# timoblak/sq-recovery

Hardware: AMD Instinct MI355X
Metric: training images/sec (256x256 depth, implicit loss) (higher is better)
Workload: dtype bf16; 1 GPU; ResNetSQ + ImplicitLoss(R=32, tau=1.5, s=260) train step, Adam; model=ResNetSQ (resnet18 backbone, 11.37M params), global_batch=64, per_gpu_batch=64, image=256x256x1, render_size=32, parallelism=dp1

## Files before the change

sq-recovery_amd/csrc/sqr_conv3.hip:

```cpp
#include <stdint.h>
#include <stdlib.h>
#include <type_traits>
#include "sqr_conv_dev.h"

namespace sqr {
namespace conv {

#ifdef SQR_STAMPS
#ifndef SQR_STAMP_MAXWG
#define SQR_STAMP_MAXWG 8192
#endif
#define SQR_STAMP_DECL unsigned long long stamp_[5] = {0, 0, 0, 0, 0};
#define SQR_STAMP(i) (stamp_[i] = wall_clock64())
#define SQR_STAMP_WRITE(tp)                                                              \
  do {                                                                                   \
    if ((tp) && threadIdx.x == 0 && blockIdx.x < SQR_STAMP_MAXWG) {                      \
      for (int i_ = 0; i_ < 5; ++i_) (tp)[2 + 8 * blockIdx.x + i_] = stamp_[i_];          \
      (tp)[2 + 8 * blockIdx.x + 5] = blockIdx.x;                                         \
    }                                                                                    \
  } while (0)
#else
#define SQR_STAMP_DECL
#define SQR_STAMP(i) ((void)0)
#define SQR_STAMP_WRITE(tp) ((void)0)
#endif

__device__ __forceinline__ int d3key(int row) { return row & 6; }

constexpr unsigned long long K20_LUT = 0xadc1f8859b07e93ull;
__device__ __forceinline__ int k20key(int row) { return (int)((K20_LUT >> (3 * (row % 20))) & 7); }

struct D3Args {
  const void* x;
  const void* w;
  void* out;
  const void* addend;
  const uint8_t* addend_mask;
  const void* bn_x;
  const uint8_t* bn_mask;
  const float* bn_mean;
  const float* bn_coef;
  void* bn_act;
  const float* in_coef;
  float* stats;
  int N, H, W, Cin, Nout;
  int iH, iW;
  int tiles_x, tiles_per_img;
  int ntm, ntn;
  int flip;
  uint32_t xbytes, wbytes;
  unsigned long long* tp;
#ifdef SQR_EXPERIMENTS
  int exp;
#endif
};

#ifdef SQR_EXPERIMENTS
#define SQR_ABL(a, bit) (((a).exp & (bit)) != 0)
#else
#define SQR_ABL(a, bit) false
#endif

__device__ __forceinline__ void dma_piece(__amdgpu_buffer_rsrc_t srd, char* dst, uint32_t voff, int soff) {
  __builtin_amdgcn_raw_ptr_buffer_load_lds(srd, (__attribute__((address_space(3))) void*)dst, 16, voff, soff, 0, 0);
}

template <int PIECES, int NW>
__device__ __forceinline__ void dma_pieces(__amdgpu_buffer_rsrc_t srd, char* dst, const uint32_t* voff, int soff,
                                           int wave) {
#pragma unroll
  for (int i = 0; i < PIECES; ++i)
    __builtin_amdgcn_raw_ptr_buffer_load_lds(srd, (__attribute__((address_space(3))) void*)(dst + ((i * NW + wave) * 8) * 128),
                                             16, voff[i], soff, 0, 0);
}

template <int BN, int WAVES_M, int WAVES_N, int TN, int NT>
__device__ __forceinline__ void stats_reduce(const float (*s1)[4], const float (*s2)[4], float* red, int wm, int wn,
                                             int fr, int fq, int tid, float* stats_row0, float* stats_row1) {
  constexpr int WN = BN / WAVES_N;
  float* r1 = red + (wm * 16 + fr) * BN + wn * WN + 4 * fq;
  float* r2 = r1 + WAVES_M * 16 * BN;
#pragma unroll
  for (int j = 0; j < TN; ++j) {
    *(f32x4*)(r1 + 16 * j) = f32x4{s1[j][0], s1[j][1], s1[j][2], s1[j][3]};
    *(f32x4*)(r2 + 16 * j) = f32x4{s2[j][0], s2[j][1], s2[j][2], s2[j][3]};
  }
  __syncthreads();
  for (int c = tid; c < 2 * BN; c += NT) {
    const int q = c / BN, col = c - q * BN;
    const float* src = red + q * WAVES_M * 16 * BN + col;
    float acc = 0.f;
#pragma unroll 8
    for (int r = 0; r < WAVES_M * 16; ++r) acc += src[r * BN];
    (q ? stats_row1 : stats_row0)[col] = acc;
  }
}

template <typename T, int BN, int WAVES_M, int WAVES_N, int TM, int TN, int NT>
__device__ __forceinline__ void tile_stats(const uint32_t (*pk)[TM][2], float* red, int wm, int wn, int fr, int fq,
                                           int tid, float* stats_row0, float* stats_row1, float* count, float bm) {
  constexpr int WN = BN / WAVES_N;
  constexpr float NG = 16.f * TM, INV_NG = 1.f / (16.f * TM);
  float* r1 = red + wm * BN + wn * WN + 4 * fq;
  float* r2 = r1 + WAVES_M * BN;
  float m[TN][4], q[TN][4];
#pragma unroll
  for (int j = 0; j < TN; ++j) {
#pragma unroll
    for (int e = 0; e < 4; ++e) {
      float v[TM];
#pragma unroll
      for (int i = 0; i < TM; ++i) v[i] = (e & 1) ? hi2f<T>(pk[j][i][e >> 1]) : lo2f<T>(pk[j][i][e >> 1]);
      const float K = row_first(v[0]);
      float sa = 0.f, sq = 0.f;
#pragma unroll
      for (int i = 0; i < TM; ++i) {
        const float d = v[i] - K;
        sa += d;
        sq = fmaf(d, d, sq);
      }
      sa = row_sum15(sa);
      sq = row_sum15(sq);
      const float sn = sa * INV_NG;
      m[j][e] = K + sn;
      q[j][e] = fmaxf(sq - sa * sn, 0.f);
    }
  }
  if (fr == 15) {
#pragma unroll
    for (int j = 0; j < TN; ++j) {
      *(f32x4*)(r1 + 16 * j) = f32x4{m[j][0], m[j][1], m[j][2], m[j][3]};
      *(f32x4*)(r2 + 16 * j) = f32x4{q[j][0], q[j][1], q[j][2], q[j][3]};
    }
  }
  __syncthreads();
  for (int col = tid; col < BN; col += NT) {
    float mean, m2;
    lane_rows_merge(red + col, red + WAVES_M * BN + col, WAVES_M, BN, NG, &mean, &m2);
    stats_row0[col] = mean;
    stats_row1[col] = m2;
  }
  if (count && tid == 0) *count = bm;
}

#ifndef SQR_D3_WINPF
#define SQR_D3_WINPF 1
#endif
template <typename T, int BM, int BN, int WAVES_M, int WAVES_N, int TW, int TH, int NWB, int IMGS = 1, int PD = 2,
          bool ACC = false, bool BNB = false, int S = 1, bool BNIN = false>
__global__ void __launch_bounds__(64 * WAVES_M * WAVES_N) conv3_kernel(D3Args a) {
  constexpr int NT = 64 * WAVES_M * WAVES_N, NW = WAVES_M * WAVES_N;
  constexpr int ROWB = 128, STAGES = PD + 1;
  constexpr int WM = BM / WAVES_M, WN = BN / WAVES_N;
  constexpr int TM = WM / 16, TN = WN / 16;
  static_assert(S == 1 || (S == 2 && IMGS == 1 && !ACC && !BNB), "stride 2: forward, one image per tile");
  constexpr int WWID = S == 1 ? TW + 2 : TW + 1;
  static_assert(!BNIN || (S == 1 && !ACC && !BNB), "apply-on-load: stride-1 forward");
  constexpr bool K20 = S == 1 && TW == 8 && !BNIN;
  constexpr int P0 = (TH + 1) * WWID, P1 = TH * WWID;
  constexpr int WRI = S == 1 ? (TH + 2) * WWID : 2 * P0 + 2 * P1, WR = IMGS * WRI;
  constexpr int WROWS = (WR + 8 * NW - 1) / (8 * NW) * (8 * NW);
  constexpr int PB = BN / (8 * NW);
  constexpr int WP = WROWS / (8 * NW);
  static_assert(BM == IMGS * TH * TW, "pixel tile");
  static_assert(PB >= 1 && PB * 8 * NW == BN, "BN must be a multiple of 8 * waves");
  constexpr int WIN = WROWS * ROWB, TILE_B = BN * ROWB;
  constexpr int LDS = NWB * WIN + STAGES * TILE_B;
  static_assert(2 * WAVES_M * 16 * BN * 4 <= LDS, "stats scratch fits the ring");
  __shared__ __attribute__((aligned(1024))) char smem[LDS + (BNIN ? 2 * 512 * 4 : 0)];
  float* const ctab = (float*)(smem + LDS);
  char* const bring = smem + NWB * WIN;
  clock_begin(a.tp);
  SQR_STAMP_DECL
  SQR_STAMP(0);

  const int tid = threadIdx.x, lane = tid & 63;
  const int wave = __builtin_amdgcn_readfirstlane(tid >> 6);
  const int wm = wave / WAVES_N, wn = wave % WAVES_N;
  const int bid = xcd_remap(blockIdx.x, gridDim.x);
  const int tile_m = bid / a.ntn, tile_n = bid - (bid / a.ntn) * a.ntn;
  const int img = (tile_m / a.tiles_per_img) * IMGS;
  const int trem = tile_m - (tile_m / a.tiles_per_img) * a.tiles_per_img;
  const int ty = trem / a.tiles_x, tx = trem - ty * a.tiles_x;
  const int h0 = ty * TH, w0 = tx * TW, n0 = tile_n * BN;

  const int fr = lane & 15, fq = lane >> 4;
  auto out_off = [&](int i) -> size_t {
    const int m = wm * WM + 16 * i + fr;
    const int ii = m / (TH * TW), mm = m - ii * (TH * TW);
    return (((size_t)(img + ii) * a.H + h0 + mm / TW) * a.W + w0 + (mm % TW)) * a.Nout + n0 + wn * WN + 4 * fq;
  };
  u32x2 av[ACC || BNB ? TN : 1][ACC || BNB ? TM : 1];
  uint32_t bmk[(BNB || ACC) ? TN : 1][(BNB || ACC) ? TM : 1];
  constexpr bool LATE = NW == 4 && TM * TN >= 16;
  auto load_av = [&]() {
    const uint16_t* ad = (const uint16_t*)(BNB ? a.bn_x : a.addend);
#pragma unroll
    for (int i = 0; i < TM; ++i) {
      const size_t o = out_off(i);
#pragma unroll
      for (int j = 0; j < TN; ++j) {
        av[j][i] = *(const u32x2*)(ad + o + 16 * j);
        if constexpr (BNB) bmk[j][i] = a.bn_coef ? 0u : a.bn_mask[(o + 16 * j) >> 3];
        if constexpr (ACC) bmk[j][i] = a.addend_mask ? a.addend_mask[(o + 16 * j) >> 3] : 0xffu;
      }
    }
  };
  if constexpr ((ACC || BNB) && !LATE) load_av();

  constexpr uint32_t kOOB = 0x80000000u;
  const int prow = lane >> 3, pslot = lane & 7;
  uint32_t wvoff[WP];
#pragma unroll
  for (int i = 0; i < WP; ++i) {
    const int r = (i * NW + wave) * 8 + prow;
    const int ls = pslot ^ (K20 ? k20key(r) : d3key(r));
    const int ii = r / WRI, rr = r - ii * WRI;
    int h, w;
    bool used = r < WR;
    if constexpr (S == 1) {
      const int wy = rr / WWID, wx = rr - wy * WWID;
      h = h0 - 1 + wy;
      w = w0 - 1 + wx;
    } else {
      const int pa = rr >= 2 * P0 ? 1 : 0;
// ... 257 lines not shown
      pk[j][i][0] = pack2<T>(acc[j][i][0], acc[j][i][1]);
      pk[j][i][1] = pack2<T>(acc[j][i][2], acc[j][i][3]);
    }
  uint32_t ak[BNB ? TN : 1][BNB ? TM : 1][2];
  if constexpr (BNB) {
    const bool bc = a.bn_coef != nullptr;
    float s1[TN][4], s2[TN][4], mu[TN][4], csc[TN][4], csh[TN][4];
#pragma unroll
    for (int j = 0; j < TN; ++j)
#pragma unroll
      for (int e = 0; e < 4; ++e) {
        const int c = n0 + wn * WN + 16 * j + 4 * fq + e;
        s1[j][e] = s2[j][e] = 0.f;
        mu[j][e] = a.bn_mean[c];
        const float* cp = bc ? a.bn_coef : a.bn_mean;
        csc[j][e] = cp[c];
        csh[j][e] = cp[bc ? a.Nout + c : c];
      }
#pragma unroll
    for (int j = 0; j < TN; ++j)
#pragma unroll
      for (int i = 0; i < TM; ++i) {
        uint32_t mb;
        if (bc) {
          mb = 0;
#pragma unroll
          for (int h = 0; h < 2; ++h) {
            const uint32_t v = pack2<T>(fmaxf(fmaf(lo2f<T>(av[j][i][h]), csc[j][2 * h], csh[j][2 * h]), 0.f),
                                        fmaxf(fmaf(hi2f<T>(av[j][i][h]), csc[j][2 * h + 1], csh[j][2 * h + 1]), 0.f));
            ak[j][i][h] = v;
            mb |= (lo2f<T>(v) > 0.f ? 1u : 0u) << (2 * h);
            mb |= (hi2f<T>(v) > 0.f ? 1u : 0u) << (2 * h + 1);
          }
        } else {
          mb = (bmk[j][i] >> ((opix[i] + 16 * j) & 4)) & 0xfu;
        }
        pk[j][i][0] &= ((mb & 1u) ? 0xffffu : 0u) | ((mb & 2u) ? 0xffff0000u : 0u);
        pk[j][i][1] &= ((mb & 4u) ? 0xffffu : 0u) | ((mb & 8u) ? 0xffff0000u : 0u);
#pragma unroll
        for (int h = 0; h < 2; ++h) {
          const float g0 = lo2f<T>(pk[j][i][h]), g1 = hi2f<T>(pk[j][i][h]);
          s1[j][2 * h] += g0;
          s2[j][2 * h] = fmaf(g0, lo2f<T>(av[j][i][h]) - mu[j][2 * h], s2[j][2 * h]);
          s1[j][2 * h + 1] += g1;
          s2[j][2 * h + 1] = fmaf(g1, hi2f<T>(av[j][i][h]) - mu[j][2 * h + 1], s2[j][2 * h + 1]);
        }
      }
    stats_reduce<BN, WAVES_M, WAVES_N, TN, NT>(s1, s2, (float*)smem, wm, wn, fr, fq, tid,
                                               a.stats + ((size_t)tile_m * 2) * a.Nout + n0,
                                               a.stats + ((size_t)tile_m * 2 + 1) * a.Nout + n0);
  }
  uint16_t* out = (uint16_t*)a.out;
  static_assert(TN % 2 == 0, "tile pairs");
  const int sw = 12 * (fq & 1);
#pragma unroll
  for (int i = 0; i < TM; ++i)
#pragma unroll
    for (int j = 0; j < TN; j += 2) {
      const auto r0 = __builtin_amdgcn_permlane16_swap(pk[j][i][0], pk[j + 1][i][0], false, false);
      const auto r1 = __builtin_amdgcn_permlane16_swap(pk[j][i][1], pk[j + 1][i][1], false, false);
      if (!SQR_ABL(a, 2)) *(u32x4*)(out + opix[i] + 16 * j + sw) = u32x4{r0[0], r1[0], r0[1], r1[1]};
      if constexpr (BNB) {
        if (a.bn_act) {
          const auto q0 = __builtin_amdgcn_permlane16_swap(ak[j][i][0], ak[j + 1][i][0], false, false);
          const auto q1 = __builtin_amdgcn_permlane16_swap(ak[j][i][1], ak[j + 1][i][1], false, false);
          *(u32x4*)((uint16_t*)a.bn_act + opix[i] + 16 * j + sw) = u32x4{q0[0], q1[0], q0[1], q1[1]};
        }
      }
    }
  if (!BNB && a.stats)
    tile_stats<T, BN, WAVES_M, WAVES_N, TM, TN, NT>(pk, (float*)smem, wm, wn, fr, fq, tid,
                                                 a.stats + ((size_t)tile_m * 2) * a.Nout + n0,
                                                 a.stats + ((size_t)tile_m * 2 + 1) * a.Nout + n0,
                                                 tile_n == 0 ? a.stats + (size_t)a.ntm * 2 * a.Nout + tile_m : nullptr,
                                                 (float)BM);
#ifdef SQR_STAMPS
  asm volatile("s_waitcnt vmcnt(0)" ::: "memory");
#endif
  SQR_STAMP(4);
  SQR_STAMP_WRITE(a.tp);
  clock_end(a.tp);
}


struct D3PArgs {
  const void* x;
  const void* w;
  void* out;
  const void* addend;
  const uint8_t* addend_mask;
  const void* bn_x;
  const uint8_t* bn_mask;
  const float* bn_mean;
  float* stats;
  const float* in_coef;
  void* in_act;
  uint8_t* in_mask;
  int H, bpi, tpb, flip;
  uint32_t xbytes, wbytes;
  unsigned long long* tp;
};

template <typename T, bool STATS, bool ACC = false, bool BNB = false, int TW = 64, int TH = 2, bool BNIN = false>
__global__ void __launch_bounds__(256) conv3p_kernel(D3PArgs a) {
  constexpr int C = 64, BN = 64, NW = 4, NT = 256, ROWB = 128;
  constexpr int WAVES_M = 2, WAVES_N = 2, WM = TH * TW / WAVES_M, WN = 32, TM = WM / 32;
  constexpr int SLOTR = (TW + 2 + 7) / 8 * 8;
  constexpr int PPR = SLOTR / 8;
  constexpr int NSLOT = TH + 2 <= 4 ? 4 : 8;
  constexpr int RING = NSLOT * SLOTR * ROWB;
  constexpr int WB = 9 * BN * ROWB;
  constexpr int WPW = 9 * BN / (8 * NW);
  constexpr int STG = TH * TW * BN * 2;
  constexpr int NST = STG / 16 / NT;
  static_assert(TW % 32 == 0 && TM * 32 == WM && WN == 32, "a wave's pixels are whole 32-pixel runs of rows");
  static_assert(STG <= WB, "the staged tile fits the weight image's region");
  static_assert(2 * WAVES_M * 32 * BN * 4 <= RING && NT * 16 * 4 <= RING, "statistics scratch fits the ring");
  static_assert(NST <= 8, "store schedule");
  static_assert(!BNIN || (STATS && !ACC && !BNB), "apply-on-load: forward launches only");
  __shared__ __attribute__((aligned(1024))) char smem[WB + RING];
  __shared__ __attribute__((aligned(16))) float bnc[BNIN ? 128 : 4];
  char* const wl = smem + RING;
  char* const ring = smem;
  char* const stg = wl;
  clock_begin(a.tp);

  const int tid = threadIdx.x, lane = tid & 63;
  const int wave = __builtin_amdgcn_readfirstlane(tid >> 6);
  const int wm = wave / WAVES_N, wn = wave % WAVES_N;
  const int prow = lane >> 3, pslot = lane & 7;
  constexpr uint32_t kOOB = 0x80000000u;
  const __amdgpu_buffer_rsrc_t xsrd = __builtin_amdgcn_make_buffer_rsrc((void*)a.x, 0, a.xbytes, 0x00020000);
  const __amdgpu_buffer_rsrc_t wsrd = __builtin_amdgcn_make_buffer_rsrc((void*)a.w, 0, a.wbytes, 0x00020000);
  const int H = a.H, ntile = a.tpb;
  const int img = blockIdx.x / a.bpi;
  const int hb = (blockIdx.x - img * a.bpi) * ntile * TH;

  constexpr int RPW = (TH * PPR + NW - 1) / NW;
  constexpr int PRW = ((TH + 2) * PPR + NW - 1) / NW;
  auto row_piece = [&](int r0, int p, uint32_t* vo, bool use = true) {
    const int j = p / PPR, part = p - j * PPR;
    const int row = r0 + j;
    const int lbase = ((row + 1) & (NSLOT - 1)) * SLOTR + part * 8;
    const int L = lbase + prow, w = part * 8 + prow - 1;
    const bool ok = use && (unsigned)row < (unsigned)H && (unsigned)w < (unsigned)TW;
    *vo = ok ? (uint32_t)((((img * H + row) * TW + w) * C) * 2 + (pslot << 4)) : kOOB;
    return L * ROWB + ((pslot ^ ((L >> 1) & 7)) << 4);
  };
  auto load_rows = [&](int r0, int nrows, u32x4* v, bool use) {
#pragma unroll
    for (int i = 0; i < PRW; ++i) {
      const int p = i * NW + wave;
      if (i < (nrows * PPR + NW - 1) / NW) {
        uint32_t vo;
        row_piece(r0, p, &vo, use && p < nrows * PPR);
        v[i] = __builtin_amdgcn_raw_buffer_load_b128(xsrd, vo, 0, 0);
      }
    }
  };
  auto load_row_piece = [&](int r0, int i, u32x4* v, bool use) {
    const int p = i * NW + wave;
    uint32_t vo;
    row_piece(r0, p, &vo, use && p < TH * PPR);
    v[i] = __builtin_amdgcn_raw_buffer_load_b128(xsrd, vo, 0, 0);
  };
  auto write_rows = [&](int r0, int nrows, const u32x4* v) {
// ... 425 lines not shown
  const int H = 2 * a.Ho, W = 2 * a.Wo;
  T* out = (T*)a.dx;
  constexpr int NIT = (HALF + 64 * NW - 1) / (64 * NW), AG = NIT < 4 ? NIT : 4;
  static_assert(NIT % AG == 0, "addend groups");
  auto piece = [&](int it, int ph, int& p, int& sl, size_t& go) {
    const int idx = tid + it * 64 * NW;
    p = idx / SL;
    sl = idx - p * SL;
    const int y = p / PX, x = p - y * PX;
    go = (((size_t)img * H + 2 * (i0 + y) + ph) * W + 2 * j0 + x) * a.C + n0 + 8 * sl;
    return idx < HALF && i0 + y < a.Ho && j0 + (x >> 1) < a.Wo;
  };
  auto load_group = [&](int it0, int ph, uint4* av) {
#pragma unroll
    for (int u = 0; u < AG; ++u) {
      int p, sl;
      size_t go;
      if (piece(it0 + u, ph, p, sl, go)) {
        if (a.addend_s2) {
          const int y = p / PX, x = p - y * PX;
          av[u] = (x & 1) ? uint4{0u, 0u, 0u, 0u}
                          : *(const uint4*)((const T*)a.addend +
                                            (((size_t)img * a.Ho + i0 + y) * a.Wo + j0 + (x >> 1)) * a.C + n0 +
                                                8 * sl);
        } else {
          av[u] = *(const uint4*)((const T*)a.addend + go);
        }
      }
    }
  };
#pragma unroll
  for (int ph = 0; ph < 2; ++ph) {
    const bool add = a.addend && !(a.addend_s2 && ph == 1);
    uint4 av[AG];
    if (add) load_group(0, ph, av);
    if (ph) __syncthreads();
#pragma unroll
    for (int pw = 0; pw < 2; ++pw)
#pragma unroll
      for (int i = 0; i < TM; ++i) {
        const int m = wm * WM + 16 * i + fr;
        const int p = (m / TW) * PX + 2 * (m % TW) + pw;
#pragma unroll
        for (int j = 0; j < TN; ++j) {
          const int n = wn * WN + 16 * j + 4 * fq;
          const int slot = (n >> 3) ^ ((p >> 1) & 7);
          store4((T*)(smem + p * (BN * 2) + slot * 16 + (n & 4) * 2), acc[2 * ph + pw][j][i]);
        }
      }
    __syncthreads();
#pragma unroll
    for (int it0 = 0; it0 < NIT; it0 += AG) {
      if (it0 && add) load_group(it0, ph, av);
#pragma unroll
      for (int u = 0; u < AG; ++u) {
        int p, sl;
        size_t go;
        if (!piece(it0 + u, ph, p, sl, go)) continue;
        uint4 v = *(const uint4*)(smem + p * (BN * 2) + ((sl ^ ((p >> 1) & 7)) << 4));
        if (add) {
          uint32_t* vv = (uint32_t*)&v;
          const uint32_t* aa = (const uint32_t*)&av[u];
#pragma unroll
          for (int e = 0; e < 4; ++e)
            vv[e] = pack2<T>(lo2f<T>(vv[e]) + lo2f<T>(aa[e]), hi2f<T>(vv[e]) + hi2f<T>(aa[e]));
        }
        *(uint4*)(out + go) = v;
      }
    }
  }
  asm volatile("s_waitcnt vmcnt(0) lgkmcnt(0)" ::: "memory");
  clock_end(a.tp);
}

__device__ __forceinline__ int psw(int y, int x) { return ((x >> 1) & 1) | ((((x >> 3) ^ y) & 1) << 1); }

template <int OFF>
__device__ __forceinline__ s16x4 ds_read_tr16_off(uint32_t addr) {
  s16x4 r;
  asm volatile("ds_read_b64_tr_b16 %0, %1 offset:%2" : "=v"(r) : "v"(addr), "n"(OFF));
  return r;
}

template <int B, int E, typename F>
__device__ __forceinline__ void static_for(F&& f) {
  if constexpr (B < E) {
    f(std::integral_constant<int, B>{});
    static_for<B + 1, E>(f);
  }
}

template <int N>
__device__ __forceinline__ void lgkm_wait() {
  static_assert(N >= 0 && N <= 15, "lgkmcnt field");
  asm volatile("s_waitcnt lgkmcnt(%0)" ::"n"(N) : "memory");
}

template <int PER>
__device__ __forceinline__ void wait_vm_chunks(int m) {
  if (m >= 2) {
    asm volatile("s_waitcnt vmcnt(%0)" ::"n"(2 * PER) : "memory");
  } else if (m == 1) {
    asm volatile("s_waitcnt vmcnt(%0)" ::"n"(PER) : "memory");
  } else {
    asm volatile("s_waitcnt vmcnt(0)" ::: "memory");
  }
}

constexpr int wg_lgkm(int j, int D, int NS, bool last) {
  int n = 0;
  for (int k = j - D + 1; k <= j - 1; ++k) {
    if (last && k + D >= NS) continue;
    n += 2 + ((k + D) % 9 == 0 ? 8 : 0);
  }
  return n > 15 ? 15 : n;
}

struct D3WArgs {
  const void* x;
  const void* dy;
  float* slab;
  int N, H, W, C, K, Ho, Wo;
  int tiles_x, chunks_per_img, nchunks, cps;
  int ntc, ntiles;
  uint32_t xbytes, dybytes;
  unsigned long long* tp;
};

template <int S, int TW, int TH>
struct WgWin {
  static constexpr int PH(int a) { return S == 1 ? TH + 2 : TH + 1 - a; }
  static constexpr int PW(int b) { return S == 1 ? TW + 2 : (b ? TW : TW + 2); }
  static constexpr int PB(int a, int b) {
    return S == 1 ? 0 : (a * 2 + b >= 1 ? PH(0) * PW(0) : 0) + (a * 2 + b >= 2 ? PH(0) * PW(1) : 0) +
                            (a * 2 + b >= 3 ? PH(1) * PW(0) : 0);
  }
  static constexpr int ROWS = S == 1 ? PH(0) * PW(0) : PB(1, 1) + PH(1) * PW(1);
  static constexpr int YO(int r) { return S == 1 ? r : r >> 1; }
  static constexpr int PA(int r) { return S == 1 ? 0 : r & 1; }
};

template <typename T, int TW, int TH, int STAGES, int S>
__global__ void __launch_bounds__(256) conv3_wgrad_kernel(D3WArgs a) {
  constexpr int NW = 4, ROWB = 128;
  constexpr int BKP = TW * TH, SUBS = BKP / 32;
  using Win = WgWin<S, TW, TH>;
  constexpr int WR = Win::ROWS;
  constexpr int WROWS = (WR + 31) / 32 * 32;
  constexpr int DP = BKP / 32, XP = WROWS / 32;
  constexpr int PER = DP + XP;
  constexpr int TILE_D = BKP * ROWB, STAGE = TILE_D + WROWS * ROWB;
  static_assert(BKP % 64 == 0, "chunk = multiple of 64 pixels");
  __shared__ __attribute__((aligned(1024))) char smem[STAGES * STAGE];

  const int tid = threadIdx.x, lane = tid & 63;
  const int wave = __builtin_amdgcn_readfirstlane(tid >> 6);
  const int bid = xcd_remap(blockIdx.x, gridDim.x);
  clock_begin(a.tp);
  SQR_STAMP_DECL
  SQR_STAMP(0);
  const int split = bid / a.ntiles, tile = bid - split * a.ntiles;
  const int k0 = (tile / a.ntc) * 64, c0 = (tile % a.ntc) * 64;
  const int ch0 = split * a.cps;
  const int nloc = min(a.nchunks - ch0, a.cps);

  constexpr uint32_t kOOB = 0x80000000u;
  const int prow = lane >> 3, pslot = lane & 7;
  uint32_t dvoff[DP];
#pragma unroll
  for (int i = 0; i < DP; ++i) {
    const int r = (i * NW + wave) * 8 + prow;
    const int lch = 2 * ((pslot >> 1) ^ psw(r / TW, r % TW)) + (pslot & 1);
    dvoff[i] = (uint32_t)((((r / TW) * a.Wo + (r % TW)) * a.K + k0 + lch * 8) * 2);
  }
// ... 207 lines not shown
  clock_end(a.tp);
}

namespace {
int g_direct = 1;
int g_deep_ring = 1;

#ifdef SQR_EXPERIMENTS
int exp_env(const char* n, int dflt) {
  const char* v = getenv(n);
  return v && *v ? atoi(v) : dflt;
}
#else
constexpr int exp_env(const char*, int dflt) { return dflt; }
#endif

int pow2_log(int x) {
  int l = 0;
  while ((1 << l) < x) ++l;
  return (1 << l) == x ? l : -1;
}

int dt16(int dtype) { return dtype == SQR_DTYPE_F16 ? 1 : 0; }

using D3Launch = void (*)(dim3 grid, hipStream_t st, const D3Args& a);
struct D3Entries {
  D3Launch plain;
  D3Launch acc;
  D3Launch bnb;
  D3Launch bnin;
};
struct D3Tile {
  int id;
  int BN, WAVES_M, WAVES_N, TW, TH, NWB, IMGS, PD;
  bool exact_bn;
  bool deep_ring;
  bool nso_faster;
  D3Entries e[2];
};
enum : unsigned { kExactBn = 1, kDeepRing = 2, kNsoFaster = 4 };
constexpr int kNoBnin = -1, kBninSamePd = 0;

template <typename T, int BN, int WM, int WN, int TW, int TH, int NWB, int IMGS, int PD, bool ACC, bool BNB, int S,
          bool BNIN>
void d3_launch(dim3 grid, hipStream_t st, const D3Args& a) {
  hipLaunchKernelGGL((conv3_kernel<T, IMGS * TH * TW, BN, WM, WN, TW, TH, NWB, IMGS, PD, ACC, BNB, S, BNIN>), grid,
                     dim3(64 * WM * WN), 0, st, a);
}
template <typename T, int BN, int WM, int WN, int TW, int TH, int NWB, int IMGS, int PD, int BNIN_PD, int S>
constexpr D3Entries d3_entries() {
  D3Entries e = {d3_launch<T, BN, WM, WN, TW, TH, NWB, IMGS, PD, false, false, S, false>, nullptr, nullptr, nullptr};
  if constexpr (S == 1) {
    e.acc = d3_launch<T, BN, WM, WN, TW, TH, NWB, IMGS, PD, true, false, S, false>;
    e.bnb = d3_launch<T, BN, WM, WN, TW, TH, NWB, IMGS, PD, false, true, S, false>;
  }
  if constexpr (BNIN_PD != kNoBnin)
    e.bnin = d3_launch<T, BN, WM, WN, TW, TH, NWB, IMGS, BNIN_PD == kBninSamePd ? PD : BNIN_PD, false, false, S, true>;
  return e;
}
template <int ID, int BN, int WM, int WN, int TW, int TH, int NWB, int IMGS, int PD, int BNIN_PD = kNoBnin, int S = 1>
constexpr D3Tile d3_tile(unsigned flags = 0) {
  return {ID, BN, WM, WN, TW, TH, NWB, IMGS, PD, (flags & kExactBn) != 0, (flags & kDeepRing) != 0,
          (flags & kNsoFaster) != 0,
          {d3_entries<bf16, BN, WM, WN, TW, TH, NWB, IMGS, PD, BNIN_PD, S>(),
           d3_entries<f16, BN, WM, WN, TW, TH, NWB, IMGS, PD, BNIN_PD, S>()}};
}

constexpr D3Tile kD3Tiles[] = {
    d3_tile<0, 64, 4, 1, 64, 4, 1, 1, 2>(kExactBn),
    d3_tile<7, 128, 4, 2, 32, 8, 2, 1, 3, 2>(kDeepRing | kNsoFaster),
    d3_tile<8, 128, 4, 2, 16, 8, 2, 1, 5, kBninSamePd>(kDeepRing | kNsoFaster),
    d3_tile<10, 64, 2, 2, 8, 8, 2, 2, 8, kBninSamePd>(kDeepRing),
    d3_tile<1, 128, 4, 2, 32, 8, 2, 1, 2, kBninSamePd>(kNsoFaster),
    d3_tile<2, 128, 4, 2, 16, 8, 2, 1, 2, kBninSamePd>(kNsoFaster),
    d3_tile<5, 64, 2, 2, 8, 8, 2, 2, 2, kBninSamePd>(),
    d3_tile<3, 128, 2, 2, 8, 8, 2, 1, 2>(),
    d3_tile<4, 64, 4, 1, 16, 16, 2, 1, 2>(),
};
constexpr D3Tile kD3S2FTiles[] = {
    d3_tile<0, 128, 4, 2, 32, 4, 1, 1, 2, kNoBnin, 2>(),
    d3_tile<1, 128, 2, 2, 16, 4, 2, 1, 2, kNoBnin, 2>(),
    d3_tile<2, 128, 2, 2, 8, 8, 2, 1, 2, kNoBnin, 2>(),
};
constexpr int kBninMaxC = 512;

bool enough_tiles(long long tiles) { return !(tiles < 128 && g_direct < 2); }

const D3Tile* pick(int N, int H, int W, int Cin, int Nout) {
  const int nch = Cin / 64;
  static const int force = exp_env("SQR_D3_CFG", -1);
  for (const D3Tile& c : kD3Tiles) {
    if (force >= 0 && c.id != force) continue;
    if (force < 0 && !g_deep_ring && c.deep_ring) continue;
    if (c.exact_bn ? Nout != c.BN : Nout % c.BN) continue;
    if (W % c.TW || H % c.TH) continue;
    if (c.IMGS > 1 && (c.TH != H || c.TW != W || N % c.IMGS)) continue;
    if (c.NWB == 1 && nch != 1) continue;
    if (!enough_tiles((long long)(N / c.IMGS) * (H / c.TH) * (W / c.TW) * (Nout / c.BN))) continue;
    return &c;
  }
  return nullptr;
}

const D3Tile* pick_s2f(int N, int Ho, int Wo, int Cin, int Nout) {
  const int nch = Cin / 64;
  static const int force = exp_env("SQR_S2F_CFG", -1);
  for (const D3Tile& c : kD3S2FTiles) {
    if (force >= 0 && c.id != force) continue;
    if ((c.NWB == 1) != (nch == 1)) continue;
    if (Nout % c.BN || Wo % c.TW || Ho % c.TH) continue;
    if (!enough_tiles((long long)N * (Ho / c.TH) * (Wo / c.TW) * (Nout / c.BN))) continue;
    return &c;
  }
  return nullptr;
}

int persist_rows(int W) { return W == 64 ? 2 : 1; }
bool persist_shape(int Cin, int Nout, int H, int W) {
  return Cin == 64 && Nout == 64 && (W == 64 || W == 128) && H % persist_rows(W) == 0;
}
}

int conv3_bnin_nso_ok(int N, int H, int W, int C, int K) {
  if (g_direct == 0 || C % 64 || K % 64 || pow2_log(W) < 0 || C > kBninMaxC) return 0;
  if (persist_shape(C, K, H, W)) return 0;
  const D3Tile* f = pick(N, H, W, C, K);
  return f && f->nso_faster && pick(N, H, W, K, C) ? 1 : 0;
}

namespace {
template <typename T, int TW, int TH>
void d3p_launch(const Conv3Call& c, dim3 grid, const D3PArgs& p) {
  const dim3 blk(256);
  if (c.bnin)
    hipLaunchKernelGGL((conv3p_kernel<T, true, false, false, TW, TH, true>), grid, blk, 0, c.st, p);
  else if (c.bnb)
    hipLaunchKernelGGL((conv3p_kernel<T, false, false, true, TW, TH>), grid, blk, 0, c.st, p);
  else if (c.stats)
    hipLaunchKernelGGL((conv3p_kernel<T, true, false, false, TW, TH>), grid, blk, 0, c.st, p);
  else if (c.addend)
    hipLaunchKernelGGL((conv3p_kernel<T, false, true, false, TW, TH>), grid, blk, 0, c.st, p);
  else
    hipLaunchKernelGGL((conv3p_kernel<T, false, false, false, TW, TH>), grid, blk, 0, c.st, p);
}

int conv3p_launch(const Conv3Call& c, size_t xbytes, size_t wbytes) {
  static int ncu = 0;
  if (!ncu) {
    int dev = 0;
    if (hipGetDevice(&dev) != hipSuccess) dev = 0;
    if (hipDeviceGetAttribute(&ncu, hipDeviceAttributeMultiprocessorCount, dev) != hipSuccess || ncu <= 0) ncu = 256;
  }
  const int tpi = c.H / persist_rows(c.W);
  int bpi = 1;
  for (int d = 1; d <= tpi; ++d)
    if (tpi % d == 0 && (long long)c.N * d <= ncu) bpi = d;
  D3PArgs p;
  p.x = c.x;
  p.w = c.w;
  p.out = c.out;
  p.addend = c.addend;
  p.addend_mask = c.addend_mask;
  p.bn_x = c.bnb ? c.bnb->x : nullptr;
  p.bn_mask = c.bnb ? c.bnb->mask : nullptr;
  p.bn_mean = c.bnb ? c.bnb->mean : nullptr;
  p.stats = c.stats;
  p.in_coef = c.bnin ? c.bnin->coef : nullptr;
  p.in_act = c.bnin ? c.bnin->act : nullptr;
  p.in_mask = c.bnin ? c.bnin->mask : nullptr;
  p.H = c.H;
  p.bpi = bpi;
  p.tpb = tpi / bpi;
  p.flip = c.flip;
  p.xbytes = (uint32_t)xbytes;
  p.wbytes = (uint32_t)wbytes;
  p.tp = probe_clock_take();
  const dim3 grid(c.N * bpi);
  if (c.stats_rows) *c.stats_rows = (int)grid.x;
  probe_begin(c.st);
  SQR_DISPATCH16(c.dtype, T, {
    if (c.W == 128) d3p_launch<T, 128, 1>(c, grid, p);
    else d3p_launch<T, 64, 2>(c, grid, p);
  });
  probe_end(c.st);
  SQR_HIP_LAUNCH_CHECK("conv3p_kernel");
  return 0;
}

D3Args d3_args(const Conv3Call& c, const D3Tile& t, int Ho, int Wo, size_t xbytes, size_t wbytes) {
  D3Args a = {};
  a.x = c.x;
  a.w = c.w;
  a.out = c.out;
  a.addend = c.addend;
  a.addend_mask = c.addend_mask;
  if (c.bnb) {
    a.bn_x = c.bnb->x;
    a.bn_mask = c.bnb->mask;
    a.bn_mean = c.bnb->mean;
    a.bn_coef = c.bnb->coef;
    a.bn_act = c.bnb->act;
  }
  a.in_coef = c.bnin ? c.bnin->coef : nullptr;
  a.stats = c.stats;
  a.N = c.N;
  a.H = Ho;
  a.W = Wo;
  a.iH = c.H;
  a.iW = c.W;
  a.Cin = c.Cin;
  a.Nout = c.Nout;
  a.tiles_x = Wo / t.TW;
  a.tiles_per_img = (Ho / t.TH) * a.tiles_x;
  a.ntm = c.N / t.IMGS * a.tiles_per_img;
  a.ntn = c.Nout / t.BN;
  a.flip = c.flip;
  a.xbytes = (uint32_t)xbytes;
  a.wbytes = (uint32_t)wbytes;
  a.tp = probe_clock_take();
#ifdef SQR_EXPERIMENTS
  a.exp = exp_env("SQR_EXP", 0);
  if (a.exp & 1) a.stats = nullptr;
#endif
  return a;
}
}

int conv3_launch(const Conv3Call& c) {
  if (c.addend_mask && (!c.addend || c.stride != 1)) return kNotHandled;
  const bool persist = persist_shape(c.Cin, c.Nout, c.H, c.W);
  if (c.bnin) {
    if (c.stride != 1 || c.flip || c.addend || c.bnb || !c.stats || (!c.bnin->act) != (!c.bnin->mask)) return kNotHandled;
    if (c.bnin->act && !persist) return kNotHandled;
  }
  if (c.bnb && c.bnb->act && !c.bnb->coef) return kNotHandled;
  if (c.bnb && c.bnb->coef && persist) return kNotHandled;
  if (g_direct == 0 || c.Cin % 64 || c.Nout % 64) return kNotHandled;
  const bool s2 = c.stride == 2;
  if (s2 ? (c.flip || c.addend || c.bnb || c.H % 2 || c.W % 2) : pow2_log(c.W) < 0) return kNotHandled;
  const int Ho = s2 ? c.H / 2 : c.H, Wo = s2 ? c.W / 2 : c.W;
  const size_t xbytes = (size_t)c.N * c.H * c.W * c.Cin * 2, wbytes = (size_t)c.Nout * 9 * c.Cin * 2;
  if (xbytes >= (1u << 31) || wbytes >= (1u << 31) || (size_t)c.N * Ho * Wo * c.Nout * 2 >= (1u << 31)) return kNotHandled;
  if (!s2 && persist) return conv3p_launch(c, xbytes, wbytes);
  const D3Tile* t = s2 ? pick_s2f(c.N, Ho, Wo, c.Cin, c.Nout) : pick(c.N, c.H, c.W, c.Cin, c.Nout);
  if (!t) return kNotHandled;
  const D3Entries& e = t->e[dt16(c.dtype)];
  if (c.bnin && (!e.bnin || c.Cin > kBninMaxC)) return kNotHandled;
  const D3Args a = d3_args(c, *t, Ho, Wo, xbytes, wbytes);
  if (c.stats_rows) *c.stats_rows = a.ntm;
  probe_begin(c.st);
  (c.bnin ? e.bnin : c.bnb ? e.bnb : c.addend ? e.acc : e.plain)(dim3(a.ntm * a.ntn), c.st, a);
  probe_end(c.st);
  SQR_HIP_LAUNCH_CHECK("conv3_kernel");
  return 0;
}

namespace {
using S2DLaunch = void (*)(dim3 grid, hipStream_t st, const D3S2Args& a);
struct S2DTile {
  int C, K, TH, TW;
  S2DLaunch e[2];
};
constexpr int kS2dBN = 64;
template <typename T, int TH, int TW, int WM, int WN, int NCH, int PD>
void s2d_launch(dim3 grid, hipStream_t st, const D3S2Args& a) {
  hipLaunchKernelGGL((conv3s2_dgrad_kernel<T, TH, TW, kS2dBN, WM, WN, NCH, PD>), grid, dim3(64 * WM * WN), 0, st, a);
}
template <int C, int K, int TH, int TW, int WM, int WN, int PD>
constexpr S2DTile s2d_tile() {
  return {C, K, TH, TW, {s2d_launch<bf16, TH, TW, WM, WN, K / 64, PD>, s2d_launch<f16, TH, TW, WM, WN, K / 64, PD>}};
}
constexpr S2DTile kS2DTiles[] = {
    s2d_tile<64, 128, 8, 32, 4, 2, 5>(),
    s2d_tile<128, 256, 4, 16, 2, 2, 3>(),
    s2d_tile<256, 512, 8, 8, 2, 2, 3>(),
};
const S2DTile* s2_pick(int Ho, int Wo, int K, int C) {
  for (const S2DTile& t : kS2DTiles)
    if (t.C == C && t.K == K) return Wo % t.TW == 0 && Ho % t.TH == 0 ? &t : nullptr;
  return nullptr;
}
}

int conv3s2_dgrad_launch(const Conv3S2DgradCall& c) {
  if (g_direct == 0) return kNotHandled;
  const S2DTile* t = s2_pick(c.Ho, c.Wo, c.K, c.C);
  if (!t) return kNotHandled;
  const size_t dybytes = (size_t)c.N * c.Ho * c.Wo * c.K * 2, wbytes = (size_t)9 * c.C * c.K * 2;
  if (dybytes >= (1u << 31) || (size_t)c.N * 4 * c.Ho * c.Wo * c.C * 2 >= (1u << 31)) return kNotHandled;
  D3S2Args a;
  a.dy = c.dy;
  a.w = c.w_cls;
  a.dx = c.dx;
  a.addend = c.addend;
  a.addend_s2 = c.addend && c.addend_s2 ? 1 : 0;
  a.N = c.N;
  a.Ho = c.Ho;
  a.Wo = c.Wo;
  a.K = c.K;
  a.C = c.C;
  a.tiles_x = c.Wo / t->TW;
  a.tiles_per_img = (c.Ho / t->TH) * a.tiles_x;
  a.ntn = c.C / kS2dBN;
  for (int i = 0; i < 4; ++i) a.cls_off[i] = c.cls_off[i];
  a.dybytes = (uint32_t)dybytes;
  a.wbytes = (uint32_t)wbytes;
  a.tp = probe_clock_take();
  probe_begin(c.st);
  t->e[dt16(c.dtype)](dim3(c.N * a.tiles_per_img * a.ntn), c.st, a);
  probe_end(c.st);
  SQR_HIP_LAUNCH_CHECK("conv3s2_dgrad_kernel");
  return 0;
}

namespace {
using D3WLaunch = void (*)(dim3 grid, hipStream_t st, const D3WArgs& a);
struct D3WTile {
  int stride, TW, TH;
  D3WLaunch e[2];
};
template <typename T, int S, int TW, int TH, int STAGES>
void d3w_launch(dim3 grid, hipStream_t st, const D3WArgs& a) {
  hipLaunchKernelGGL((conv3_wgrad_kernel<T, TW, TH, STAGES, S>), grid, dim3(256), 0, st, a);
}
template <int S, int TW, int TH, int STAGES>
constexpr D3WTile d3w_tile() {
// ... 93 lines not shown
```

Baseline: 28170 images/s.

## Add dedicated stride-2 forward conv kernel with tap-ordered weight ring and multi-tile waves

Adds a specialized stride-2 3x3 forward convolution kernel that loads even/odd-row input windows once per channel chunk, streams weight taps through a deeper ring in a reordered tap sequence, and prefetches the next tap's activation fragments before the barrier. A workgroup can walk several M tiles in sequence (TPW), and BN statistics can be emitted as several rows per tile (SROWS), which needs a generalized tile_stats. Stride-2 calls without BN-on-load now go to this kernel before the older generic path. The cost is extra tile configurations, more code complexity, and possible mismatches in the stats row layout that consumers must handle through stats_rows.

Result: no change. 28340 images/s (median of 6 runs) (+0.6%).

```diff
diff --git a/sq-recovery_amd/csrc/sqr_conv3.hip b/sq-recovery_amd/csrc/sqr_conv3.hip
--- a/sq-recovery_amd/csrc/sqr_conv3.hip
+++ b/sq-recovery_amd/csrc/sqr_conv3.hip
@@ -96,9 +96,10 @@
   }
 }
 
-template <typename T, int BN, int WAVES_M, int WAVES_N, int TM, int TN, int NT>
+template <typename T, int BN, int WAVES_M, int WAVES_N, int TM, int TN, int NT, int ROWS = 1>
 __device__ __forceinline__ void tile_stats(const uint32_t (*pk)[TM][2], float* red, int wm, int wn, int fr, int fq,
-                                           int tid, float* stats_row0, float* stats_row1, float* count, float bm) {
+                                           int tid, float* stats_row0, float* stats_row1, float* count, float bm,
+                                           size_t row_step = 0, int count_step = 0) {
   constexpr int WN = BN / WAVES_N;
   constexpr float NG = 16.f * TM, INV_NG = 1.f / (16.f * TM);
   float* r1 = red + wm * BN + wn * WN + 4 * fq;
@@ -134,13 +135,26 @@
     }
   }
   __syncthreads();
-  for (int col = tid; col < BN; col += NT) {
-    float mean, m2;
-    lane_rows_merge(red + col, red + WAVES_M * BN + col, WAVES_M, BN, NG, &mean, &m2);
-    stats_row0[col] = mean;
-    stats_row1[col] = m2;
-  }
-  if (count && tid == 0) *count = bm;
+  if constexpr (ROWS == 1) {
+    for (int col = tid; col < BN; col += NT) {
+      float mean, m2;
+      lane_rows_merge(red + col, red + WAVES_M * BN + col, WAVES_M, BN, NG, &mean, &m2);
+      stats_row0[col] = mean;
+      stats_row1[col] = m2;
+    }
+    if (count && tid == 0) *count = bm;
+  } else {
+    constexpr int G = WAVES_M / ROWS;
+    static_assert(G * ROWS == WAVES_M, "whole wave rows per statistics row");
+    for (int c = tid; c < ROWS * BN; c += NT) {
+      const int g = c / BN, col = c - g * BN;
+      float mean, m2;
+      lane_rows_merge(red + g * G * BN + col, red + (WAVES_M + g * G) * BN + col, G, BN, NG, &mean, &m2);
+      stats_row0[g * row_step + col] = mean;
+      stats_row1[g * row_step + col] = m2;
+    }
+    if (count && tid < ROWS) count[tid * count_step] = bm;
+  }
 }
 
 #ifndef SQR_D3_WINPF
@@ -564,6 +578,251 @@
   clock_end(a.tp);
 }
 
+template <int B, int E, typename F>
+__device__ __forceinline__ void static_for(F&& f) {
+  if constexpr (B < E) {
+    f(std::integral_constant<int, B>{});
+    static_for<B + 1, E>(f);
+  }
+}
+
+constexpr int s2f_tap(int s) { return s < 3 ? s : s < 6 ? s + 3 : s - 3; }
+constexpr int s2f_wait(int s, int PB, int PD, int WPX, int WPY) {
+  int n = PB * (PD - 1);
+  for (int j = s + 2 - PD; j <= s; ++j) {
+    const int sj = (j + 9) % 9;
+    n += sj == 0 ? WPY : sj == 6 ? WPX : 0;
+  }
+  if (s == 4 && n > 5 * PB) n = 5 * PB;
+  if (s == 8 && n > 3 * PB) n = 3 * PB;
+  return n;
+}
+
+template <typename T, int BN, int WAVES_M, int WAVES_N, int TW, int TH, int IMGS, int PD, int TPW, int SROWS>
+__global__ void __launch_bounds__(64 * WAVES_M * WAVES_N) conv3s2f_kernel(D3Args a) {
+  constexpr int NT = 64 * WAVES_M * WAVES_N, NW = WAVES_M * WAVES_N;
+  constexpr int ROWB = 128, STAGES = PD + 1;
+  constexpr int BM = IMGS * TH * TW;
+  constexpr int WM = BM / WAVES_M, WN = BN / WAVES_N;
+  constexpr int TM = WM / 16, TN = WN / 16;
+  constexpr int WWID = TW + 1;
+  constexpr int P0 = (TH + 1) * WWID, P1 = TH * WWID;
+  constexpr int XR = IMGS * 2 * P0, YR = IMGS * 2 * P1;
+  constexpr int XROWS = (XR + 8 * NW - 1) / (8 * NW) * (8 * NW), YROWS = (YR + 8 * NW - 1) / (8 * NW) * (8 * NW);
+  constexpr int WPX = XROWS / (8 * NW), WPY = YROWS / (8 * NW);
+  constexpr int PB = BN / (8 * NW);
+  constexpr int XB = XROWS * ROWB, YB = YROWS * ROWB, TILE_B = BN * ROWB;
+  constexpr int SCR = 2 * WAVES_M * BN * 4;
+  constexpr int LDS = XB + YB + STAGES * TILE_B + (TPW > 1 ? SCR : 0);
+  static_assert(LDS <= 160 * 1024, "the tile fits the LDS");
+  static_assert(SCR <= STAGES * TILE_B, "stats scratch fits the ring");
+  static_assert(TM * 16 * WAVES_M == BM && TN * 16 * WAVES_N == BN && TN % 2 == 0, "wave tiles");
+  static_assert((TH * TW) % 16 == 0, "a fragment's 16 pixels lie in one image");
+  static_assert(SROWS == 1 || (IMGS == 1 && TH % SROWS == 0 && WAVES_M % SROWS == 0 && (TH / SROWS) * TW == WM * (WAVES_M / SROWS)),
+                "a statistics row is whole tile rows and whole wave rows");
+  static_assert(PB >= 1 && PB * 8 * NW == BN, "BN must be a multiple of 8 * waves");
+  static_assert(PD >= 2 && PD <= 8, "ring depth");
+  static_assert(PB * (PD - 1) + WPX + WPY <= 63, "vmcnt range");
+  __shared__ __attribute__((aligned(1024))) char smem[LDS];
+  char* const bring = smem + XB + YB;
+  float* const scr = (float*)(TPW > 1 ? bring + STAGES * TILE_B : bring);
+  clock_begin(a.tp);
+
+  const int tid = threadIdx.x, lane = tid & 63;
+  const int wave = __builtin_amdgcn_readfirstlane(tid >> 6);
+  const int wm = wave / WAVES_N, wn = wave % WAVES_N;
+  const int bid = xcd_remap(blockIdx.x, gridDim.x);
+  const int pm = bid / a.ntn, tile_n = bid - pm * a.ntn;
+  const int n0 = tile_n * BN;
+  const int tm0 = pm * TPW;
+  const int ntl = min(TPW, a.ntm - tm0);
+  const int fr = lane & 15, fq = lane >> 4;
+
+  constexpr uint32_t kOOB = 0x80000000u;
+  const int prow = lane >> 3, pslot = lane & 7;
+  uint32_t xv[WPX], yv[WPY];
+  auto win_voff = [&](int tile_m) {
+    const int img = (tile_m / a.tiles_per_img) * IMGS;
+    const int trem = tile_m - (tile_m / a.tiles_per_img) * a.tiles_per_img;
+    const int ty = trem / a.tiles_x, tx = trem - ty * a.tiles_x;
+    const int h0 = ty * TH, w0 = tx * TW;
+    auto off = [&](int r, int PR, int pa) -> uint32_t {
+      const int ls = pslot ^ d3key(r);
+      const int ii = r / (2 * PR), rr = r - ii * (2 * PR);
+      const int pb = rr >= PR ? 1 : 0, pr = rr - pb * PR;
+      const int py = pr / WWID, px = pr - py * WWID;
+      const int h = 2 * h0 - 1 + 2 * py + pa, w = 2 * w0 - 1 + 2 * px + pb;
+      const bool ok = ii < IMGS && (pb == 0 || px < TW) && (unsigned)h < (unsigned)a.iH && (unsigned)w < (unsigned)a.iW;
+      return ok ? (uint32_t)(((((img + ii) * a.iH + h) * a.iW + w) * a.Cin) * 2 + ls * 16) : kOOB;
+    };
+#pragma unroll
+    for (int i = 0; i < WPX; ++i) xv[i] = off((i * NW + wave) * 8 + prow, P0, 0);
+#pragma unroll
+    for (int i = 0; i < WPY; ++i) yv[i] = off((i * NW + wave) * 8 + prow, P1, 1);
+  };
+  win_voff(tm0);
+  uint32_t bvoff[PB];
+#pragma unroll
+  for (int i = 0; i < PB; ++i) {
+    const int r = (i * NW + wave) * 8 + prow;
+    bvoff[i] = (uint32_t)(((n0 + r) * 9 * a.Cin) * 2 + (pslot ^ d3key(r)) * 16);
+  }
+  const __amdgpu_buffer_rsrc_t xsrd = __builtin_amdgcn_make_buffer_rsrc((void*)a.x, 0, a.xbytes, 0x00020000);
+  const __amdgpu_buffer_rsrc_t wsrd = __builtin_amdgcn_make_buffer_rsrc((void*)a.w, 0, a.wbytes, 0x00020000);
+
+  int qbx[TM], qby[TM];
+#pragma unroll
+  for (int i = 0; i < TM; ++i) {
+    const int m = wm * WM + 16 * i + fr;
+    const int ii = m / (TH * TW), mm = m - ii * (TH * TW);
+    qbx[i] = ii * 2 * P0 + (mm / TW) * WWID + (mm % TW);
+    qby[i] = ii * 2 * P1 + (mm / TW) * WWID + (mm % TW);
+  }
+  int poff[TN];
+#pragma unroll
+  for (int j = 0; j < TN; ++j) {
+    const int row = wn * WN + 16 * j + fr;
+    poff[j] = row * ROWB + ((fq ^ d3key(row)) << 4);
+  }
+  auto tap_qoff = [&](auto sc, int* qo) {
+    constexpr int tap = s2f_tap(decltype(sc)::value), r = tap / 3, c3 = tap % 3;
+    constexpr bool odd = r == 1;
+    constexpr int toff = (c3 & 1) * (odd ? P1 : P0) + (r >> 1) * WWID + (c3 >> 1);
+#pragma unroll
+    for (int i = 0; i < TM; ++i) {
+      int row = (odd ? qby[i] : qbx[i]) + toff;
+      asm volatile("" : "+v"(row));
+      qo[i] = (odd ? XB : 0) + row * ROWB + ((fq ^ d3key(row)) << 4);
+    }
+  };
+
+  const int nch = a.Cin >> 6;
+  const int total = ntl * nch * 9;
+  auto issue_w = [&](int q, int sq, int cq) {
+    dma_pieces<PB, NW>(wsrd, bring + (q % STAGES) * TILE_B, bvoff,
+                       __builtin_amdgcn_readfirstlane((s2f_tap(sq) * a.Cin + cq * 64) * 2), wave);
+  };
+  if constexpr (PD < 3) dma_pieces<WPX, NW>(xsrd, smem, xv, 0, wave);
+  static_for<0, PD>([&](auto qc) __attribute__((always_inline)) {
+    constexpr int q = decltype(qc)::value;
+    if constexpr (q == PD - 3) dma_pieces<WPX, NW>(xsrd, smem, xv, 0, wave);
+    issue_w(q, q, 0);
+  });
+  asm volatile("s_waitcnt vmcnt(%0) lgkmcnt(0)" ::"n"(PB * (PD - 1 < 3 ? PD - 1 : 3)) : "memory");
+  __builtin_amdgcn_s_barrier();
+
+  f32x4 acc[TN][TM];
+  int qoff_n[TM];
+  V8<T> qn[TM];
+  uint16_t* const out = (uint16_t*)a.out;
+  int gq = 0;
+  for (int tl = 0; tl < ntl; ++tl) {
+#pragma unroll
+    for (int j = 0; j < TN; ++j)
+#pragma unroll
+      for (int i = 0; i < TM; ++i) acc[j][i] = f32x4{0.f, 0.f, 0.f, 0.f};
+    const int tile_m = tm0 + tl;
+    const bool last_tile = tl + 1 >= ntl;
+    for (int cc = 0; cc < nch; ++cc) {
+      const bool last_chunk = cc + 1 >= nch;
+      static_for<0, 9>([&](auto sc) __attribute__((always_inline)) {
+        constexpr int s = decltype(sc)::value;
+        if constexpr (s == 0)
+          dma_pieces<WPY, NW>(xsrd, smem + XB, yv, __builtin_amdgcn_readfirstlane(cc * 128), wave);
+        if constexpr (s == 6) {
+          int nc = cc + 1;
+          if (last_chunk) {
+            nc = last_tile ? cc : 0;
+            if (!last_tile) win_voff(tile_m + 1);
+          }
+          dma_pieces<WPX, NW>(xsrd, smem, xv, __builtin_amdgcn_readfirstlane(nc * 128), wave);
+        }
+        const char* bst = bring + (gq % STAGES) * TILE_B;
+        int qoff[TM];
+        if constexpr (s == 0) {
+          tap_qoff(sc, qoff);
+        } else {
+#pragma unroll
+          for (int i = 0; i < TM; ++i) qoff[i] = qoff_n[i];
+        }
+#pragma unroll
+        for (int sub = 0; sub < 2; ++sub) {
+          V8<T> pf[TN], qf[TM];
+#pragma unroll
+          for (int j = 0; j < TN; ++j) pf[j] = *(const V8<T>*)(bst + (poff[j] ^ (sub << 6)));
+#pragma unroll
+          for (int i = 0; i < TM; ++i) qf[i] = sub == 0 && s > 0 ? qn[i] : *(const V8<T>*)(smem + (qoff[i] ^ (sub << 6)));
+#pragma unroll
+          for (int j = 0; j < TN; ++j)
+#pragma unroll
+            for (int i = 0; i < TM; ++i) acc[j][i] = mfma(pf[j], qf[i], acc[j][i]);
+        }
+        {
+          constexpr int sq = (s + PD) % 9, adv = (s + PD) / 9;
+          int cq = cc + adv;
+          bool past = false;
+          if (adv && cq >= nch) {
+            cq = 0;
+            past = last_tile;
+          }
+          if (past) issue_w(total - 1, 8, nch - 1);
+          else issue_w(gq + PD, sq, cq);
+        }
+        constexpr bool pre = s < 8;
+        if constexpr (pre) {
+          tap_qoff(std::integral_constant<int, s + 1>{}, qoff_n);
+#pragma unroll
+          for (int i = 0; i < TM; ++i) qn[i] = *(const V8<T>*)(smem + qoff_n[i]);
+        }
+        asm volatile("s_waitcnt vmcnt(%0) lgkmcnt(%1)" ::"n"(s2f_wait(s, PB, PD, WPX, WPY)), "n"(pre ? TM : 0) : "memory");
+        __builtin_amdgcn_s_barrier();
+        ++gq;
+      });
+    }
+    if constexpr (TPW == 1) {
+      asm volatile("s_waitcnt vmcnt(0) lgkmcnt(0)" ::: "memory");
+      __builtin_amdgcn_s_barrier();
+    }
+
+    const int img = (tile_m / a.tiles_per_img) * IMGS;
+    const int trem = tile_m - (tile_m / a.tiles_per_img) * a.tiles_per_img;
+    const int ty = trem / a.tiles_x, tx = trem - ty * a.tiles_x;
+    const int h0 = ty * TH, w0 = tx * TW;
+    uint32_t pk[TN][TM][2];
+#pragma unroll
+    for (int j = 0; j < TN; ++j)
+#pragma unroll
+      for (int i = 0; i < TM; ++i) {
+        pk[j][i][0] = pack2<T>(acc[j][i][0], acc[j][i][1]);
+        pk[j][i][1] = pack2<T>(acc[j][i][2], acc[j][i][3]);
+      }
+    const int sw = 12 * (fq & 1);
+#pragma unroll
+    for (int i = 0; i < TM; ++i) {
+      const int m = wm * WM + 16 * i + fr;
+      const int ii = m / (TH * TW), mm = m - ii * (TH * TW);
+      const size_t opix =
+          (((size_t)(img + ii) * a.H + h0 + mm / TW) * a.W + w0 + (mm % TW)) * a.Nout + n0 + wn * WN + 4 * fq;
+#pragma unroll
+      for (int j = 0; j < TN; j += 2) {
+        const auto r0 = __builtin_amdgcn_permlane16_swap(pk[j][i][0], pk[j + 1][i][0], false, false);
+        const auto r1 = __builtin_amdgcn_permlane16_swap(pk[j][i][1], pk[j + 1][i][1], false, false);
+        *(u32x4*)(out + opix + 16 * j + sw) = u32x4{r0[0], r1[0], r0[1], r1[1]};
+      }
+    }
+    if (a.stats) {
+      const int row = SROWS * tile_m - (SROWS - 1) * tx;
+      tile_stats<T, BN, WAVES_M, WAVES_N, TM, TN, NT, SROWS>(
+          pk, scr, wm, wn, fr, fq, tid, a.stats + ((size_t)row * 2) * a.Nout + n0,
+          a.stats + ((size_t)row * 2 + 1) * a.Nout + n0,
+          tile_n == 0 ? a.stats + (size_t)SROWS * a.ntm * 2 * a.Nout + row : nullptr, (float)(BM / SROWS),
+          (size_t)a.tiles_x * 2 * a.Nout, a.tiles_x);
+    }
+  }
+  asm volatile("s_waitcnt vmcnt(0)" ::: "memory");
+  clock_end(a.tp);
+}
+
 
 struct D3PArgs {
   const void* x;
@@ -1155,14 +1414,6 @@
   return r;
 }
 
-template <int B, int E, typename F>
-__device__ __forceinline__ void static_for(F&& f) {
-  if constexpr (B < E) {
-    f(std::integral_constant<int, B>{});
-    static_for<B + 1, E>(f);
-  }
-}
-
 template <int N>
 __device__ __forceinline__ void lgkm_wait() {
   static_assert(N >= 0 && N <= 15, "lgkmcnt field");
@@ -1536,6 +1787,27 @@
     d3_tile<1, 128, 2, 2, 16, 4, 2, 1, 2, kNoBnin, 2>(),
     d3_tile<2, 128, 2, 2, 8, 8, 2, 1, 2, kNoBnin, 2>(),
 };
+struct S2FTile {
+  int id;
+  int BN, TW, TH, IMGS, TPW, SROWS;
+  bool one_chunk;
+  D3Launch e[2];
+};
+template <typename T, int BN, int WM, int WN, int TW, int TH, int IMGS, int PD, int TPW, int SROWS>
+void s2f_launch(dim3 grid, hipStream_t st, const D3Args& a) {
+  hipLaunchKernelGGL((conv3s2f_kernel<T, BN, WM, WN, TW, TH, IMGS, PD, TPW, SROWS>), grid, dim3(64 * WM * WN), 0, st, a);
+}
+template <int ID, int BN, int WM, int WN, int TW, int TH, int IMGS, int PD, int TPW, int SROWS>
+constexpr S2FTile s2f_tile(bool one_chunk) {
+  return {ID, BN, TW, TH, IMGS, TPW, SROWS, one_chunk,
+          {s2f_launch<bf16, BN, WM, WN, TW, TH, IMGS, PD, TPW, SROWS>,
+           s2f_launch<f16, BN, WM, WN, TW, TH, IMGS, PD, TPW, SROWS>}};
+}
+constexpr S2FTile kS2FTiles[] = {
+    s2f_tile<3, 128, 4, 2, 32, 4, 1, 3, 2, 1>(true),
+    s2f_tile<4, 128, 4, 2, 16, 8, 1, 4, 1, 2>(false),
+    s2f_tile<5, 64, 2, 2, 8, 8, 2, 8, 1, 1>(false),
+};
 constexpr int kBninMaxC = 512;
 
 bool enough_tiles(long long tiles) { return !(tiles < 128 && g_direct < 2); }
@@ -1564,6 +1836,20 @@
     if ((c.NWB == 1) != (nch == 1)) continue;
     if (Nout % c.BN || Wo % c.TW || Ho % c.TH) continue;
     if (!enough_tiles((long long)N * (Ho / c.TH) * (Wo / c.TW) * (Nout / c.BN))) continue;
+    return &c;
+  }
+  return nullptr;
+}
+
+const S2FTile* pick_s2f128(int N, int Ho, int Wo, int Cin, int Nout) {
+  static const int force = exp_env("SQR_S2F_CFG", -1);
+  for (const S2FTile& c : kS2FTiles) {
+    if (force >= 0 && c.id != force) continue;
+    if (c.one_chunk != (Cin == 64)) continue;
+    if (Nout % c.BN || Wo % c.TW || Ho % c.TH) continue;
+    if (c.IMGS > 1 && (c.TH != Ho || c.TW != Wo || N % c.IMGS)) continue;
+    const long long ntm = (long long)(N / c.IMGS) * (Ho / c.TH) * (Wo / c.TW);
+    if (!enough_tiles((ntm + c.TPW - 1) / c.TPW * (Nout / c.BN))) continue;
     return &c;
   }
   return nullptr;
@@ -1641,7 +1927,8 @@
   return 0;
 }
 
-D3Args d3_args(const Conv3Call& c, const D3Tile& t, int Ho, int Wo, size_t xbytes, size_t wbytes) {
+template <typename Tile>
+D3Args d3_args(const Conv3Call& c, const Tile& t, int Ho, int Wo, size_t xbytes, size_t wbytes) {
   D3Args a = {};
   a.x = c.x;
   a.w = c.w;
@@ -1696,6 +1983,17 @@
   const size_t xbytes = (size_t)c.N * c.H * c.W * c.Cin * 2, wbytes = (size_t)c.Nout * 9 * c.Cin * 2;
   if (xbytes >= (1u << 31) || wbytes >= (1u << 31) || (size_t)c.N * Ho * Wo * c.Nout * 2 >= (1u << 31)) return kNotHandled;
   if (!s2 && persist) return conv3p_launch(c, xbytes, wbytes);
+  if (s2 && !c.bnin) {
+    if (const S2FTile* t = pick_s2f128(c.N, Ho, Wo, c.Cin, c.Nout)) {
+      const D3Args a = d3_args(c, *t, Ho, Wo, xbytes, wbytes);
+      if (c.stats_rows) *c.stats_rows = a.ntm * t->SROWS;
+      probe_begin(c.st);
+      t->e[dt16(c.dtype)](dim3((a.ntm + t->TPW - 1) / t->TPW * a.ntn), c.st, a);
+      probe_end(c.st);
+      SQR_HIP_LAUNCH_CHECK("conv3s2f_kernel");
+      return 0;
+    }
+  }
   const D3Tile* t = s2 ? pick_s2f(c.N, Ho, Wo, c.Cin, c.Nout) : pick(c.N, c.H, c.W, c.Cin, c.Nout);
   if (!t) return kNotHandled;
   const D3Entries& e = t->e[dt16(c.dtype)];
```
